# aarchiiive/diff-unet-amos

Measured on AMD Instinct MI355X. Metric: denoised voxel-steps/sec on 96^3 16-class AMOS patches, higher is better.
Workload: dtype f16

## Files before the change

diff_unet_amos_amd/csrc/common.hpp:

```cpp
#pragma once
#include <hip/hip_runtime.h>
#include <stdint.h>

namespace dua {
struct LdsAttr { const void* fn; int bytes; };
void register_lds_attrs(const LdsAttr* list, int n);
int ensure_prepared();
int device_cus();
struct LdsAttrs {
  template <int N> explicit LdsAttrs(const LdsAttr (&list)[N]) { register_lds_attrs(list, N); }
};


using f16 = _Float16;
typedef f16 f16x8 __attribute__((ext_vector_type(8)));
typedef f16 f16x4 __attribute__((ext_vector_type(4)));
typedef float f32x4 __attribute__((ext_vector_type(4)));
typedef float f32x16 __attribute__((ext_vector_type(16)));

enum : int { DT_F32 = 0, DT_F16 = 1 };

template <typename T> struct Elem;
template <> struct Elem<f16> {
  static constexpr int EPG = 8;
  using Frag = f16x8;
};
template <> struct Elem<float> {
  static constexpr int EPG = 4;
  using Frag = f32x4;
};

__device__ __forceinline__ void mma32(f32x16& acc, const f16x8& a, const f16x8& b) {
  acc = __builtin_amdgcn_mfma_f32_32x32x16_f16(a, b, acc, 0, 0, 0);
}
__device__ __forceinline__ void mma32(f32x16& acc, const f32x4& a, const f32x4& b) {
  acc = __builtin_amdgcn_mfma_f32_32x32x2f32(a[0], b[0], acc, 0, 0, 0);
  acc = __builtin_amdgcn_mfma_f32_32x32x2f32(a[1], b[1], acc, 0, 0, 0);
  acc = __builtin_amdgcn_mfma_f32_32x32x2f32(a[2], b[2], acc, 0, 0, 0);
  acc = __builtin_amdgcn_mfma_f32_32x32x2f32(a[3], b[3], acc, 0, 0, 0);
}

__device__ __forceinline__ float gelu_erf(float x) {
  const float z = fabsf(x) * 0.70710678118654752f;
  const float t = __builtin_amdgcn_rcpf(fmaf(0.3275911f, z, 1.f));
  float p = fmaf(t, 1.061405429f, -1.453152027f);
  p = fmaf(p, t, 1.421413741f);
  p = fmaf(p, t, -0.284496736f);
  p = fmaf(p, t, 0.254829592f);
  const float e = 1.f - p * t * __expf(-z * z);
  return 0.5f * x * (1.f + copysignf(e, x));
}

__device__ __forceinline__ float other_half(float v) {
  const auto pr = __builtin_amdgcn_permlane32_swap(__float_as_uint(v), __float_as_uint(v), false, false);
  return __uint_as_float((threadIdx.x & 32) ? pr[0] : pr[1]);
}

__device__ __forceinline__ long chan_off(bool blk, long v, int c, int stride, long nvox) {
  return blk ? ((long)(c >> 4) * nvox + v) * 16 + (c & 15) : v * stride + c;
}

__device__ __forceinline__ int acc_row(int i, int h) { return (i & 3) + 8 * (i >> 2) + 4 * h; }

__device__ __forceinline__ int xcd_remap(int bid, int n) {
  int q = n >> 3, r = n & 7, x = bid & 7, j = bid >> 3;
  return (x < r ? x * (q + 1) : r * (q + 1) + (x - r) * q) + j;
}

__device__ __forceinline__ void wide_tile_origin(int bid, int ntiles, int tiles_h, int tiles_w, int& d0, int& h0, int& w0) {
  const int per_slab = tiles_h * tiles_w;
  const int tile = xcd_remap(bid, ntiles);
  const int td = tile / per_slab, rem = tile - td * per_slab, th = rem / tiles_w, tw = rem - th * tiles_w;
  d0 = td * 8; h0 = th * 8; w0 = tw * 8;
}

__device__ __forceinline__ void lds_dma_16(const void* src_lane, unsigned lds_dst) {
  unsigned keep;
  asm volatile("s_mov_b32 %0, m0\n\ts_mov_b32 m0, %2\n\ts_nop 0\n\tglobal_load_lds_dwordx4 %1, off\n\ts_mov_b32 m0, %0"
               : "=&s"(keep) : "v"(src_lane), "s"(__builtin_amdgcn_readfirstlane(lds_dst)) : "memory");
}
__device__ __forceinline__ void lds_dma_16_m0_unsaved(const void* src_lane, unsigned lds_dst) {
  asm volatile("s_mov_b32 m0, %1\n\ts_nop 0\n\tglobal_load_lds_dwordx4 %0, off" : : "v"(src_lane), "s"(__builtin_amdgcn_readfirstlane(lds_dst)) : "memory");
}

constexpr int STAT_REPLICAS = 8;

using stat_t = long long;
constexpr int STAT_WORDS = 4;
constexpr double STAT_FRAC = 17592186044416.0;

struct InXform {
  const stat_t* stats;
  const float* gamma;
  const float* beta;
  const float* add;
  double inv_count;
  int add_stride, c_pad;
  float eps, slope;
};

__device__ __forceinline__ void stats_words_value(const stat_t (&w)[STAT_WORDS], double& S, double& Q) {
  S = (double)w[0] + (double)w[1] * (1.0 / STAT_FRAC);
  Q = (double)w[2] + (double)w[3] * (1.0 / STAT_FRAC);
}

__device__ __forceinline__ void stats_read(const stat_t* stats, int n, int c_pad, int c, double& S, double& Q) {
  stat_t w[STAT_WORDS] = {0, 0, 0, 0};
#pragma unroll
  for (int r = 0; r < STAT_REPLICAS; ++r) {
    const stat_t* p = stats + ((long)n * STAT_REPLICAS + r) * STAT_WORDS * c_pad + c;
#pragma unroll
    for (int k = 0; k < STAT_WORDS; ++k) w[k] += p[(long)k * c_pad];
  }
  stats_words_value(w, S, Q);
}

__device__ __forceinline__ void stats_words_to_sums(const stat_t (&v)[2 * STAT_WORDS], double& S, double& Q) {
  stat_t w[STAT_WORDS];
#pragma unroll
  for (int k = 0; k < STAT_WORDS; ++k) {
    w[k] = v[k] + v[STAT_WORDS + k];
    w[k] += __shfl_xor(w[k], 16);
    w[k] += __shfl_xor(w[k], 32);
  }
  stats_words_value(w, S, Q);
}

__device__ __forceinline__ void stats_read_wave16(const stat_t* stats, int n, int c_pad, int c, double& S, double& Q) {
  const int part = (threadIdx.x & 63) >> 4;
  const stat_t* p = stats + ((long)n * STAT_REPLICAS + 2 * part) * STAT_WORDS * c_pad + c;
  stat_t v[2 * STAT_WORDS];
#pragma unroll
  for (int k = 0; k < 2 * STAT_WORDS; ++k) v[k] = p[(long)k * c_pad];
#ifdef DUA_STATS_F64
  S = __longlong_as_double(v[0]) + __longlong_as_double(v[STAT_WORDS]);
  Q = __longlong_as_double(v[2]) + __longlong_as_double(v[STAT_WORDS + 2]);
  S += __shfl_xor(S, 16); S += __shfl_xor(S, 32);
  Q += __shfl_xor(Q, 16); Q += __shfl_xor(Q, 32);
#else
  stats_words_to_sums(v, S, Q);
#endif
}

__device__ __forceinline__ void norm_mean_rstd(double S, double Q, double inv_count, float eps, double& mean, float& rstd) {
  mean = S * inv_count;
  double var = Q * inv_count - mean * mean;
  var = var > 0 ? var : 0;
  rstd = (float)(1.0 / sqrt(var + (double)eps));
}
__device__ __forceinline__ void norm_scale_shift(double S, double Q, double inv_count, float eps, float gamma, float beta,
                                                 float& scale, float& shift) {
  double mean;
  float rstd;
  norm_mean_rstd(S, Q, inv_count, eps, mean, rstd);
  scale = gamma * rstd;
  shift = beta - (float)mean * scale;
}

__device__ __forceinline__ void xform_preamble(const InXform& xf, int n, int C, float* sc, float* sh, float* ad,
                                               int c_begin = 0) {
  if (!xf.stats) {
    for (int c = c_begin + threadIdx.x; c < C; c += blockDim.x) {
      sc[c] = 1.f; sh[c] = 0.f;
      ad[c] = xf.add ? xf.add[(long)n * xf.add_stride + c] : 0.f;
    }
    return;
  }
  const int lane = threadIdx.x & 63, wave = threadIdx.x >> 6, nw = blockDim.x >> 6;
  constexpr int UN = 4;
  for (int c0 = c_begin + wave * 16; c0 < C; c0 += UN * nw * 16) {
    double S[UN], Q[UN];
    float gam[UN], bet[UN], add[UN];
    int cc[UN];
#pragma unroll
    for (int u = 0; u < UN; ++u) {
      const int c = c0 + u * nw * 16 + (lane & 15);
      cc[u] = c < C ? c : C - 1;
      gam[u] = xf.gamma[cc[u]]; bet[u] = xf.beta[cc[u]];
      add[u] = xf.add ? xf.add[(long)n * xf.add_stride + cc[u]] : 0.f;
    }
#pragma unroll
    for (int u = 0; u < UN; ++u) {
      S[u] = 0; Q[u] = 0;
      if (c0 + u * nw * 16 < C) stats_read_wave16(xf.stats, n, xf.c_pad, cc[u], S[u], Q[u]);
    }
    const int part = lane >> 4;
    double Sm = S[0], Qm = Q[0];
    float gm = gam[0], bm = bet[0], am = add[0];
#pragma unroll
    for (int u = 1; u < UN; ++u)
      if (part == u) { Sm = S[u]; Qm = Q[u]; gm = gam[u]; bm = bet[u]; am = add[u]; }
    const int c = c0 + part * nw * 16 + (lane & 15);
    float g, b;
    norm_scale_shift(Sm, Qm, xf.inv_count, xf.eps, gm, bm, g, b);
    if (c0 + part * nw * 16 < C && c < C) {
      sc[c] = g;
      sh[c] = b;
      ad[c] = am;
    }
  }
}

}
#include "../../include/dua_hip.h"
namespace dua {
static inline InXform make_xform(const dua_in_norm* in, int C) {
  InXform x{};
  if (in && in->stats) {
    x.stats = in->stats; x.gamma = in->gamma; x.beta = in->beta; x.add = in->add;
    x.add_stride = in->add_stride > 0 ? in->add_stride : C;
    x.c_pad = in->c_pad; x.eps = in->eps;
    x.inv_count = in->count > 0 ? 1.0 / (double)in->count : 0.0;
  }
  x.slope = in ? in->slope : 0.f;
  return x;
}

__device__ __forceinline__ void stats_add(stat_t* stats, int n, int c_pad, int replica, int c, double S, double Q) {
  unsigned long long* p = (unsigned long long*)stats + ((long)n * STAT_REPLICAS + replica) * STAT_WORDS * c_pad + c;
#ifdef DUA_STATS_F64
  unsafeAtomicAdd((double*)p, S);
  unsafeAtomicAdd((double*)(p + 2L * c_pad), Q);
  return;
#endif
  constexpr double LIM = 4.0e18;
  constexpr double POISON = 140737488355328.0;
  if (!(fabs(S) < LIM) || !(fabs(Q) < LIM)) { S = POISON; Q = -POISON; }
  const double Si = rint(S), Qi = rint(Q);
  __hip_atomic_fetch_add(p, (unsigned long long)(long long)Si, __ATOMIC_RELAXED, __HIP_MEMORY_SCOPE_SYSTEM);
  __hip_atomic_fetch_add(p + c_pad, (unsigned long long)(long long)rint((S - Si) * STAT_FRAC), __ATOMIC_RELAXED, __HIP_MEMORY_SCOPE_SYSTEM);
  __hip_atomic_fetch_add(p + 2L * c_pad, (unsigned long long)(long long)Qi, __ATOMIC_RELAXED, __HIP_MEMORY_SCOPE_SYSTEM);
  __hip_atomic_fetch_add(p + 3L * c_pad, (unsigned long long)(long long)rint((Q - Qi) * STAT_FRAC), __ATOMIC_RELAXED, __HIP_MEMORY_SCOPE_SYSTEM);
}

template <typename T>
__device__ __forceinline__ void xform_prep(float* sc, float* sh, float* ad, float* sn, float slope) {
  if constexpr (sizeof(T) == 2) {
#pragma unroll
    for (int e = 0; e < Elem<T>::EPG; ++e) {
      sn[e] = slope * sc[e];
      const float b = sh[e] + ad[e];
      ad[e] = fmaf(slope, sh[e], ad[e]);
      sh[e] = b;
    }
  }
}

typedef unsigned u32x4_t __attribute__((ext_vector_type(4)));
__device__ __forceinline__ u32x4_t xform_frag_mix(u32x4_t x, const float* a, const float* b, const float* an, const float* bn) {
  u32x4_t p, n, r;
#pragma unroll
  for (int j = 0; j < 4; ++j) asm("v_fma_mixlo_f16 %0, %1, %2, %3 op_sel_hi:[1,0,0]" : "=v"(p[j]) : "v"(x[j]), "v"(a[2 * j]), "v"(b[2 * j]));
#pragma unroll
  for (int j = 0; j < 4; ++j) asm("v_fma_mixlo_f16 %0, %1, %2, %3 op_sel_hi:[1,0,0]" : "=v"(n[j]) : "v"(x[j]), "v"(an[2 * j]), "v"(bn[2 * j]));
#pragma unroll
  for (int j = 0; j < 4; ++j)
    asm("v_fma_mixhi_f16 %0, %1, %2, %3 op_sel:[1,0,0] op_sel_hi:[1,0,0]" : "+v"(p[j]) : "v"(x[j]), "v"(a[2 * j + 1]), "v"(b[2 * j + 1]));
#pragma unroll
  for (int j = 0; j < 4; ++j)
    asm("v_fma_mixhi_f16 %0, %1, %2, %3 op_sel:[1,0,0] op_sel_hi:[1,0,0]" : "+v"(n[j]) : "v"(x[j]), "v"(an[2 * j + 1]), "v"(bn[2 * j + 1]));
#pragma unroll
  for (int j = 0; j < 4; ++j) asm("v_pk_max_f16 %0, %1, %2" : "=v"(r[j]) : "v"(p[j]), "v"(n[j]));
  return r;
}

template <typename T>
__device__ __forceinline__ typename Elem<T>::Frag xform_frag(typename Elem<T>::Frag v, const float* sc, const float* sh,
                                                               const float* ad, const float* sn, float slope) {
  constexpr int E = Elem<T>::EPG;
  typename Elem<T>::Frag o;
  if constexpr (sizeof(T) == 2) {
    o = __builtin_bit_cast(typename Elem<T>::Frag, xform_frag_mix(__builtin_bit_cast(u32x4_t, v), sc, sh, sn, ad));
  } else {
#pragma unroll
    for (int j = 0; j < E; ++j) {
      float y = fmaf((float)v[j], sc[j], sh[j]);
      y = y > 0.f ? y : y * slope;
      o[j] = (T)(y + ad[j]);
    }
  }
  return o;
}

}
```

diff_unet_amos_amd/csrc/deconv.hip:

```cpp
#include "common.hpp"
#include "../../include/dua_hip.h"
#include "conv3_form.hpp"

namespace dua {



struct DeconvArgs {
  const void* x; const void* w; const float* bias; void* y;
  InXform xf;
  int N, D, H, W;
  int Cin, Cin_stride, Cin_off, Cout, Cout_stride, Cout_off;
  int nchunks, nct, lds_base;
  int out_blk;
  int Do, Ho, Wo;
  int pad;
};

template <typename F>
__device__ __forceinline__ void pad_copies(const DeconvArgs& a, long ov, F&& st) {
  const long hw = (long)a.Ho * a.Wo;
  const int od = (int)(ov / hw), oh = (int)((ov / a.Wo) % a.Ho), ow = (int)(ov % a.Wo);
  const int e = ((a.Do & 1) && od == a.Do - 2 ? 4 : 0) | ((a.Ho & 1) && oh == a.Ho - 2 ? 2 : 0) | ((a.Wo & 1) && ow == a.Wo - 2 ? 1 : 0);
  for (int c = 1; c < 8; ++c)
    if ((c & e) == c) st(ov + ((c & 4) ? hw : 0) + ((c & 2) ? a.Wo : 0) + (c & 1));
}

template <typename T>
__global__ __launch_bounds__(256) void deconv_k2s2_kernel(DeconvArgs a) {
  using namespace dc;
  using Frag = typename Elem<T>::Frag;
  constexpr int EPG = Elem<T>::EPG;
  constexpr int CK = KG * EPG;
  constexpr int OS = BN * (int)sizeof(T) + 16;
  extern __shared__ __attribute__((aligned(16))) char smem[];
  char* alds = smem;
  char* wlds = smem + A_BYTES;
  float* xsc = (float*)(smem + a.lds_base);
  float* xsh = xsc + a.nchunks * CK;
  float* xad = xsh + a.nchunks * CK;

  const int tid = threadIdx.x, lane = tid & 63, wave = tid >> 6, r = lane & 31, hh = lane >> 5;
  const long vox = (long)a.D * a.H * a.W;
  const long v0 = (long)blockIdx.x * TM;
  const int tap = blockIdx.y / a.nct, ct = blockIdx.y % a.nct, n = blockIdx.z;
  const T* xin = (const T*)a.x + (long)n * vox * a.Cin_stride + a.Cin_off;
  const char* wsrc = (const char*)a.w + ((long)tap * a.nct + ct) * a.nchunks * W_BYTES;

  f32x16 acc[2][2];
#pragma unroll
  for (int m = 0; m < 2; ++m)
#pragma unroll
    for (int q = 0; q < 2; ++q)
#pragma unroll
      for (int i = 0; i < 16; ++i) acc[m][q][i] = 0.f;

  const int kg_t = tid & 3;
  if (a.xf.stats != nullptr) xform_preamble(a.xf, n, a.Cin, xsc, xsh, xad);
  Frag pa[4];
  f32x4 pw;
  auto load_chunk = [&](int ch) {
    const int c0 = ch * CK + kg_t * EPG;
    const bool cok = c0 < a.Cin;
#pragma unroll
    for (int j = 0; j < 4; ++j) {
      const long v = v0 + (tid >> 2) + 64 * j;
      if (v < vox && cok) pa[j] = *(const Frag*)(xin + v * a.Cin_stride + c0);
      else
#pragma unroll
        for (int e = 0; e < EPG; ++e) pa[j][e] = (T)0.f;
    }
    pw = *(const f32x4*)(wsrc + (long)ch * W_BYTES + tid * 16);
  };
  load_chunk(0);
  for (int ch = 0; ch < a.nchunks; ++ch) {
    __syncthreads();
    const int c0 = ch * CK + kg_t * EPG;
    const bool xf = a.xf.stats != nullptr && c0 < a.Cin;
    float sc[EPG], sh[EPG], ad[EPG], sn[EPG];
    if (xf) {
#pragma unroll
      for (int e = 0; e < EPG; ++e) { sc[e] = xsc[c0 + e]; sh[e] = xsh[c0 + e]; ad[e] = xad[c0 + e]; }
      xform_prep<T>(sc, sh, ad, sn, a.xf.slope);
    }
#pragma unroll
    for (int j = 0; j < 4; ++j) {
      const int vl = (tid >> 2) + 64 * j;
      Frag f = pa[j];
      if (xf && v0 + vl < vox) f = xform_frag<T>(f, sc, sh, ad, sn, a.xf.slope);
      *(Frag*)(alds + vl * VS + kg_t * 16) = f;
    }
    *(f32x4*)(wlds + tid * 16) = pw;
    __syncthreads();
    if (ch + 1 < a.nchunks) load_chunk(ch + 1);
#pragma unroll
    for (int ks = 0; ks < KG / 2; ++ks) {
      Frag a0 = *(const Frag*)(alds + (wave * 64 + r) * VS + (2 * ks + hh) * 16);
      Frag a1 = *(const Frag*)(alds + (wave * 64 + 32 + r) * VS + (2 * ks + hh) * 16);
      Frag b0 = *(const Frag*)(wlds + ((2 * ks + hh) * BN + r) * 16);
      Frag b1 = *(const Frag*)(wlds + ((2 * ks + hh) * BN + 32 + r) * 16);
      mma32(acc[0][0], a0, b0);
      mma32(acc[0][1], a0, b1);
      mma32(acc[1][0], a1, b0);
      mma32(acc[1][1], a1, b1);
    }
  }
  __syncthreads();
  char* ot = smem + wave * 64 * OS;
#pragma unroll
  for (int q = 0; q < 2; ++q) {
    const int co = q * 32 + r;
    const float bq = a.bias[ct * BN + co];
#pragma unroll
    for (int m = 0; m < 2; ++m)
#pragma unroll
      for (int i = 0; i < 16; ++i)
        *(T*)(ot + (m * 32 + acc_row(i, hh)) * OS + co * (int)sizeof(T)) = (T)(acc[m][q][i] + bq);
  }
  __syncthreads();
  constexpr int GPV = BN / EPG, VPI = 64 / GPV;
  const int ti = tap >> 2, tj = (tap >> 1) & 1, tk = tap & 1;
  const int H2 = a.Ho, W2 = a.Wo;
  T* yout = (T*)a.y + (long)n * a.Do * H2 * W2 * a.Cout_stride + a.Cout_off + ct * BN;
#pragma unroll
  for (int it = 0; it < 64 / VPI; ++it) {
    const int vl = it * VPI + lane / GPV, cg = lane % GPV;
    const long v = v0 + wave * 64 + vl;
    if (v < vox && ct * BN + cg * EPG < a.Cout) {
      const int w = (int)(v % a.W); const long t = v / a.W;
      const int h = (int)(t % a.H), d = (int)(t / a.H);
      const long ov = ((long)(2 * d + ti) * H2 + (2 * h + tj)) * W2 + (2 * w + tk);
      const Frag o = *(const Frag*)(ot + vl * OS + cg * 16);
      *(Frag*)(yout + ov * a.Cout_stride + cg * EPG) = o;
      if (a.pad) pad_copies(a, ov, [&](long c) { *(Frag*)(yout + c * a.Cout_stride + cg * EPG) = o; });
    }
  }
}

template <typename T>
__global__ __launch_bounds__(256, 2) void deconv_k2s2_ksplit_kernel(DeconvArgs a) {
  using namespace dc;
  using namespace dcs;
  using Frag = typename Elem<T>::Frag;
  constexpr int EPG = Elem<T>::EPG;
  constexpr int CK = KG * EPG;
  extern __shared__ __attribute__((aligned(16))) char smem[];
  float* xsc = (float*)(smem + RED);
  float* xsh = xsc + a.nchunks * CK;
  float* xad = xsh + a.nchunks * CK;

  const int tid = threadIdx.x, lane = tid & 63, wave = tid >> 6, r = lane & 31, hh = lane >> 5;
  const long vox = (long)a.D * a.H * a.W;
  const long v0 = (long)blockIdx.x * TMS;
  const int tap = blockIdx.y / a.nct, ct = blockIdx.y % a.nct, n = blockIdx.z;
  const T* xin = (const T*)a.x + (long)n * vox * a.Cin_stride + a.Cin_off;
  const char* wsrc = (const char*)a.w + ((long)tap * a.nct + ct) * a.nchunks * W_BYTES;
  char* alds = smem + wave * STAGE;
  char* wlds = alds + TMS * VS;
  const int kg_t = lane & 3;
  const bool fused = a.xf.stats != nullptr;

  Frag pa[MC][4];
  f32x4 pw[MC][4];
#pragma unroll
  for (int c = 0; c < MC; ++c) {
    const int ch = wave + 4 * c;
    const int c0 = ch * CK + kg_t * EPG;
    const bool cok = ch < a.nchunks && c0 < a.Cin;
#pragma unroll
    for (int j = 0; j < 4; ++j) {
      const long v = v0 + (lane >> 2) + 16 * j;
      pa[c][j] = *(const Frag*)(xin + (v < vox && cok ? v * a.Cin_stride + c0 : 0));
      pw[c][j] = *(const f32x4*)(wsrc + (ch < a.nchunks ? (long)ch * W_BYTES + (lane + 64 * j) * 16 : 0));
    }
  }
  if (fused) xform_preamble(a.xf, n, a.Cin, xsc, xsh, xad);
  __syncthreads();

  f32x16 acc[2][2];
#pragma unroll
  for (int m = 0; m < 2; ++m)
#pragma unroll
    for (int q = 0; q < 2; ++q)
#pragma unroll
      for (int i = 0; i < 16; ++i) acc[m][q][i] = 0.f;
#pragma unroll
  for (int c = 0; c < MC; ++c) {
    const int ch = wave + 4 * c;
    if (ch >= a.nchunks) break;
    const int c0 = ch * CK + kg_t * EPG;
    const bool cok = c0 < a.Cin;
    float sc[EPG], sh[EPG], ad[EPG], sn[EPG];
    if (fused && cok) {
#pragma unroll
      for (int e = 0; e < EPG; ++e) { sc[e] = xsc[c0 + e]; sh[e] = xsh[c0 + e]; ad[e] = xad[c0 + e]; }
      xform_prep<T>(sc, sh, ad, sn, a.xf.slope);
    }
#pragma unroll
    for (int j = 0; j < 4; ++j) {
      const int vl = (lane >> 2) + 16 * j;
      const bool ok = v0 + vl < vox && cok;
      Frag f = pa[c][j];
      if (fused && cok) f = xform_frag<T>(f, sc, sh, ad, sn, a.xf.slope);
#pragma unroll
      for (int e = 0; e < EPG; ++e) f[e] = ok ? f[e] : (T)0.f;
      *(Frag*)(alds + vl * VS + kg_t * 16) = f;
      *(f32x4*)(wlds + (lane + 64 * j) * 16) = pw[c][j];
    }
    __builtin_amdgcn_fence(__ATOMIC_RELEASE, "wavefront");
    __builtin_amdgcn_wave_barrier();
    __builtin_amdgcn_fence(__ATOMIC_ACQUIRE, "wavefront");
#pragma unroll
    for (int ks = 0; ks < KG / 2; ++ks) {
      const Frag a0 = *(const Frag*)(alds + r * VS + (2 * ks + hh) * 16);
      const Frag a1 = *(const Frag*)(alds + (32 + r) * VS + (2 * ks + hh) * 16);
      const Frag b0 = *(const Frag*)(wlds + ((2 * ks + hh) * BN + r) * 16);
      const Frag b1 = *(const Frag*)(wlds + ((2 * ks + hh) * BN + 32 + r) * 16);
      mma32(acc[0][0], a0, b0);
      mma32(acc[0][1], a0, b1);
      mma32(acc[1][0], a1, b0);
      mma32(acc[1][1], a1, b1);
    }
    __builtin_amdgcn_fence(__ATOMIC_RELEASE, "wavefront");
    __builtin_amdgcn_wave_barrier();
    __builtin_amdgcn_fence(__ATOMIC_ACQUIRE, "wavefront");
  }
  __syncthreads();
  float* red = (float*)(smem + wave * TMS * RS);
#pragma unroll
  for (int m = 0; m < 2; ++m)
#pragma unroll
    for (int q = 0; q < 2; ++q)
#pragma unroll
      for (int i = 0; i < 16; ++i) red[(m * 32 + acc_row(i, hh)) * (RS / 4) + q * 32 + r] = acc[m][q][i];
  __syncthreads();
  const int ti = tap >> 2, tj = (tap >> 1) & 1, tk = tap & 1;
  const int H2 = a.Ho, W2 = a.Wo;
  T* yout = (T*)a.y + (long)n * a.Do * H2 * W2 * a.Cout_stride + a.Cout_off + ct * BN;
#pragma unroll
  for (int it = 0; it < 2; ++it) {
    const int item = tid + 256 * it, vl = item >> 3, cg = item & 7;
    float o[8];
#pragma unroll
    for (int e = 0; e < 8; ++e) o[e] = 0.f;
#pragma unroll
    for (int w = 0; w < 4; ++w) {
      const float* p = (const float*)(smem + w * TMS * RS) + vl * (RS / 4) + cg * 8;
      const f32x4 lo = *(const f32x4*)p, hi = *(const f32x4*)(p + 4);
#pragma unroll
      for (int e = 0; e < 4; ++e) { o[e] += lo[e]; o[4 + e] += hi[e]; }
    }
    const long v = v0 + vl;
    if (v < vox && ct * BN + cg * 8 < a.Cout) {
      const int w = (int)(v % a.W); const long t = v / a.W;
      const int h = (int)(t % a.H), d = (int)(t / a.H);
      const long ov = ((long)(2 * d + ti) * H2 + (2 * h + tj)) * W2 + (2 * w + tk);
      T* dst = yout + ov * a.Cout_stride + cg * 8;
      if constexpr (sizeof(T) == 2) {
        Frag f;
#pragma unroll
        for (int e = 0; e < 8; ++e) f[e] = (T)(o[e] + a.bias[ct * BN + cg * 8 + e]);
        *(Frag*)dst = f;
        if (a.pad) pad_copies(a, ov, [&](long c) { *(Frag*)(yout + c * a.Cout_stride + cg * 8) = f; });
      } else {
#pragma unroll
        for (int g = 0; g < 2; ++g) {
          Frag f;
#pragma unroll
          for (int e = 0; e < 4; ++e) f[e] = (T)(o[4 * g + e] + a.bias[ct * BN + cg * 8 + 4 * g + e]);
          *(Frag*)(dst + 4 * g) = f;
          if (a.pad) pad_copies(a, ov, [&](long c) { *(Frag*)(yout + c * a.Cout_stride + cg * 8 + 4 * g) = f; });
        }
      }
    }
  }
}

template <typename T, int MBLK>
__global__ __launch_bounds__(256) void deconv_k2s2_alltaps_kernel(DeconvArgs a) {
  using namespace dc;
  constexpr int TM = 64 * MBLK * 2, WR = 32 * MBLK;
  using Frag = typename Elem<T>::Frag;
  constexpr int EPG = Elem<T>::EPG;
  constexpr int CK = KG * EPG;
  constexpr int RB = 32 * (int)sizeof(T) + 16;
  constexpr int GPV = 32 / EPG, VPI = 64 / GPV, NST = 2 * WR / VPI;
  extern __shared__ __attribute__((aligned(16))) char smem[];
  const int VSA = a.nchunks * 64 + 16;
  char* alds = smem;
  char* wlds = alds + TM * VSA;
  char* stg = wlds + 4 * a.nchunks * W_BYTES;
  float* xsc = (float*)(stg + 2 * TM * RB);
  float* xsh = xsc + a.nchunks * CK;
  float* xad = xsh + a.nchunks * CK;

  const int tid = threadIdx.x, lane = tid & 63, wave = tid >> 6, r = lane & 31, hh = lane >> 5;
  const long vox = (long)a.D * a.H * a.W;
  const long v0 = (long)blockIdx.x * TM;
  const int ct = blockIdx.y, n = blockIdx.z;
  const T* xin = (const T*)a.x + (long)n * vox * a.Cin_stride + a.Cin_off;
  const int wtap = a.nchunks * W_BYTES;
  const char* wsrc = (const char*)a.w + (long)ct * wtap;
  const int kg_t = tid & 3;

  constexpr int MCH = 4;
  Frag f[MCH][TM / 64];
#pragma unroll
  for (int ch = 0; ch < MCH; ++ch) {
    const int c0 = ch * CK + kg_t * EPG;
    const bool cok = ch < a.nchunks && c0 < a.Cin;
#pragma unroll
    for (int j = 0; j < TM / 64; ++j) {
      const long v = v0 + (tid >> 2) + 64 * j;
      f[ch][j] = *(const Frag*)(xin + (v < vox && cok ? v * a.Cin_stride + c0 : 0));
    }
  }
  f32x4 wn[2][MCH];
  auto load_pair = [&](int tp) {
#pragma unroll
    for (int tk = 0; tk < 2; ++tk)
#pragma unroll
      for (int j = 0; j < MCH; ++j)
        wn[tk][j] = *(const f32x4*)(wsrc + (long)(2 * tp + tk) * a.nct * wtap + (j < a.nchunks ? (tid + 256 * j) * 16 : 0));
  };
  auto store_pair = [&](int tp) {
#pragma unroll
    for (int tk = 0; tk < 2; ++tk)
#pragma unroll
      for (int j = 0; j < MCH; ++j)
        if (j < a.nchunks) *(f32x4*)(wlds + ((tp & 1) * 2 + tk) * wtap + (tid + 256 * j) * 16) = wn[tk][j];
  };
  load_pair(0);
  if (a.xf.stats != nullptr) {
    xform_preamble(a.xf, n, a.Cin, xsc, xsh, xad);
    __syncthreads();
  }
#pragma unroll
  for (int ch = 0; ch < MCH; ++ch) {
    if (ch >= a.nchunks) break;
    const int c0 = ch * CK + kg_t * EPG;
    const bool cok = c0 < a.Cin;
    const bool xf = a.xf.stats != nullptr && cok;
    float sc[EPG], sh[EPG], ad[EPG], sn[EPG];
    if (xf) {
#pragma unroll
      for (int e = 0; e < EPG; ++e) { sc[e] = xsc[c0 + e]; sh[e] = xsh[c0 + e]; ad[e] = xad[c0 + e]; }
      xform_prep<T>(sc, sh, ad, sn, a.xf.slope);
    }
#pragma unroll
    for (int j = 0; j < TM / 64; ++j) {
      const int vl = (tid >> 2) + 64 * j;
      const bool ok = v0 + vl < vox && cok;
      Frag g = f[ch][j];
      if (xf) g = xform_frag<T>(g, sc, sh, ad, sn, a.xf.slope);
#pragma unroll
      for (int e = 0; e < EPG; ++e) g[e] = ok ? g[e] : (T)0.f;
      *(Frag*)(alds + vl * VSA + ch * 64 + kg_t * 16) = g;
    }
  }
  store_pair(0);
  __syncthreads();

  const int H2 = a.Ho, W2 = a.Wo;
  const long ovox = (long)a.Do * H2 * W2;
  T* yout = (T*)a.y + (long)n * ovox * a.Cout_stride;
  const float bq0 = a.bias[ct * BN + r], bq1 = a.bias[ct * BN + 32 + r];
  char* ot = stg + wave * 2 * WR * RB;
  int ovb[NST];
#pragma unroll
  for (int it = 0; it < NST; ++it) {
    const int j = it * VPI + lane / GPV;
    const long v = v0 + wave * WR + (j >> 1);
    const int vi = (int)(v < vox ? v : 0);
    const int w = vi % a.W, t = vi / a.W, h = t % a.H, d = t / a.H;
    ovb[it] = v < vox ? ((2 * d) * H2 + 2 * h) * W2 + 2 * w + (j & 1) : -1;
  }
  load_pair(1);
  for (int tp = 0; tp < 4; ++tp) {
    f32x16 acc[2][MBLK][2];
#pragma unroll
    for (int tk = 0; tk < 2; ++tk) {
#pragma unroll
      for (int m = 0; m < MBLK; ++m)
#pragma unroll
        for (int i = 0; i < 16; ++i) { acc[tk][m][0][i] = bq0; acc[tk][m][1][i] = bq1; }
      const char* wb = wlds + ((tp & 1) * 2 + tk) * wtap;
      for (int ch = 0; ch < a.nchunks; ++ch) {
#pragma unroll
        for (int ks = 0; ks < KG / 2; ++ks) {
          const Frag b0 = *(const Frag*)(wb + ch * W_BYTES + ((2 * ks + hh) * BN + r) * 16);
          const Frag b1 = *(const Frag*)(wb + ch * W_BYTES + ((2 * ks + hh) * BN + 32 + r) * 16);
#pragma unroll
          for (int m = 0; m < MBLK; ++m) {
            const Frag am = *(const Frag*)(alds + (wave * WR + m * 32 + r) * VSA + ch * 64 + (2 * ks + hh) * 16);
            mma32(acc[tk][m][0], am, b0);
            mma32(acc[tk][m][1], am, b1);
          }
        }
      }
    }
    if (tp < 3) store_pair(tp + 1);
    if (tp < 2) load_pair(tp + 2);
    const int toff = ((tp >> 1) * H2 + (tp & 1)) * W2;
#pragma unroll
    for (int q = 0; q < 2; ++q) {
#pragma unroll
      for (int tk = 0; tk < 2; ++tk)
#pragma unroll
        for (int m = 0; m < MBLK; ++m)
#pragma unroll
          for (int i = 0; i < 16; ++i)
            *(T*)(ot + (2 * (m * 32 + acc_row(i, hh)) + tk) * RB + r * (int)sizeof(T)) = (T)acc[tk][m][q][i];
      __builtin_amdgcn_wave_barrier();
#pragma unroll
      for (int it = 0; it < NST; ++it) {
        const int j = it * VPI + lane / GPV, cg = lane % GPV;
        if (ovb[it] >= 0 && ct * BN + q * 32 + cg * EPG < a.Cout) {
          const Frag o = *(const Frag*)(ot + j * RB + cg * 16);
          const int c0 = a.Cout_off + ct * BN + q * 32 + cg * EPG;
          *(Frag*)(yout + chan_off(a.out_blk, ovb[it] + toff, c0, a.Cout_stride, ovox)) = o;
          if (a.pad) pad_copies(a, ovb[it] + toff, [&](long c) { *(Frag*)(yout + chan_off(a.out_blk, c, c0, a.Cout_stride, ovox)) = o; });
        }
      }
      __builtin_amdgcn_wave_barrier();
    }
    __syncthreads();
  }
}

struct DeconvResArgs {
  DeconvArgs base;
  const void* xs; const void* ws; stat_t* stats;
  int Cs, Cs_stride, Cs_off, cout_pad;
};

template <int NSK>
__global__ __launch_bounds__(256, 2) void deconv_k2s2_res_kernel(DeconvResArgs ra) {
  using namespace dc;
  using T = f16;
  const DeconvArgs& a = ra.base;
  constexpr int TM = 128, WR = 32, EPG = 8;
  using Frag = f16x8;
  constexpr int RB = 32 * 2 + 16;
  constexpr int GPV = 4, VPI = 16, NST = 2 * WR / VPI;
  extern __shared__ __attribute__((aligned(16))) char smem[];
  const int VSA = a.nchunks * 64 + 16;
  char* alds = smem;
  char* wlds = alds + TM * VSA;
  char* stg = wlds + 4 * a.nchunks * W_BYTES;
  char* skw = stg + 2 * TM * RB;

  const int tid = threadIdx.x, lane = tid & 63, wave = tid >> 6, r = lane & 31, hh = lane >> 5;
  const long vox = (long)a.D * a.H * a.W;
  const long v0 = (long)blockIdx.x * TM;
  const int ct = blockIdx.y, n = blockIdx.z;
  const T* xin = (const T*)a.x + (long)n * vox * a.Cin_stride + a.Cin_off;
  const int wtap = a.nchunks * W_BYTES;
  const char* wsrc = (const char*)a.w + (long)ct * wtap;
  const int kg_t = tid & 3;
  const int H2 = 2 * a.H, W2 = 2 * a.W;
  const T* xsk = (const T*)ra.xs + (long)n * vox * 8 * ra.Cs_stride + ra.Cs_off;

  constexpr int MCH = 4;
  Frag f[MCH][TM / 64];
#pragma unroll
  for (int ch = 0; ch < MCH; ++ch) {
    const int c0 = ch * 32 + kg_t * EPG;
    const bool cok = ch < a.nchunks && c0 < a.Cin;
#pragma unroll
    for (int j = 0; j < TM / 64; ++j) {
      const long v = v0 + (tid >> 2) + 64 * j;
      f[ch][j] = *(const Frag*)(xin + (v < vox && cok ? v * a.Cin_stride + c0 : 0));
    }
  }
  f32x4 wn[2][MCH];
  auto load_pair = [&](int tp) {
#pragma unroll
    for (int tk = 0; tk < 2; ++tk)
#pragma unroll
// ... 261 lines not shown
```

diff_unet_amos_amd/csrc/instnorm.hip:

```cpp
#include "common.hpp"
#include "../../include/dua_hip.h"

namespace dua {

__global__ void instnorm_finalize_kernel(InXform xf, int C, float* scale, float* shift) {
  extern __shared__ float sm[];
  const int n = blockIdx.x;
  xform_preamble(xf, n, C, sm, sm + C, sm + 2 * C);
  __syncthreads();
  for (int c = threadIdx.x; c < C; c += blockDim.x) { scale[n * C + c] = sm[c]; shift[n * C + c] = sm[C + c]; }
}

template <typename T, bool POOL, bool EMB, bool ODD = false>
__global__ __launch_bounds__(256) void materialize_kernel(const T* __restrict__ raw, int C, int raw_stride,
                                                          InXform xf,
                                                          const T* __restrict__ emb, int emb_stride, T* __restrict__ out,
                                                          int out_stride, int out_off, T* __restrict__ pooled,
                                                          int pool_stride, int D, int H, int W, long total, int out_blk) {
  using Frag = typename Elem<T>::Frag;
  constexpr int EPG = Elem<T>::EPG;
  extern __shared__ float sm[];
  const int gpc = C / EPG;
  const int n = blockIdx.y;
  const float slope = xf.slope;
  xform_preamble(xf, n, C, sm, sm + C, sm + 2 * C);
  __syncthreads();
  const long vox_n = (long)D * H * W;
  const bool fixed = 256 % gpc == 0;
  float sc[EPG], sh[EPG], ad[EPG];
  if (fixed) {
    const int cg = threadIdx.x % gpc;
#pragma unroll
    for (int e = 0; e < EPG; ++e) { sc[e] = sm[cg * EPG + e]; sh[e] = sm[C + cg * EPG + e]; ad[e] = sm[2 * C + cg * EPG + e]; }
  }
  for (long it = blockIdx.x * 256L + threadIdx.x; it < total; it += (long)gridDim.x * 256) {
    const int cg = (int)(it % gpc);
    long v = it / gpc;
    if (!fixed) {
#pragma unroll
      for (int e = 0; e < EPG; ++e) { sc[e] = sm[cg * EPG + e]; sh[e] = sm[C + cg * EPG + e]; ad[e] = sm[2 * C + cg * EPG + e]; }
    }
    if constexpr (!POOL) {
      const long gv = n * vox_n + v;
      Frag x = *(const Frag*)(raw + gv * raw_stride + cg * EPG);
      Frag o;
      Frag ev;
      if constexpr (EMB) ev = *(const Frag*)(emb + gv * emb_stride + cg * EPG);
#pragma unroll
      for (int e = 0; e < EPG; ++e) {
        float y = fmaf((float)x[e], sc[e], sh[e]);
        y = (y > 0.f ? y : y * slope) + ad[e];
        if constexpr (EMB) y += (float)ev[e];
        o[e] = (T)y;
      }
      *(Frag*)(out + n * vox_n * out_stride + chan_off(out_blk, v, out_off + cg * EPG, out_stride, vox_n)) = o;
    } else {
      const int W2 = W >> 1, H2 = H >> 1;
      const int WB = ODD ? (W + 1) >> 1 : W2, HB = ODD ? (H + 1) >> 1 : H2;
      const int pw = (int)(v % WB); v /= WB;
      const int ph = (int)(v % HB); const int pd = (int)(v / HB);
      float mx[EPG];
#pragma unroll
      for (int e = 0; e < EPG; ++e) mx[e] = -INFINITY;
      long gvk[8];
      bool okk[8];
      Frag xk[8], evk[EMB ? 8 : 1];
#pragma unroll
      for (int k = 0; k < 8; ++k) {
        const int d = 2 * pd + (k >> 2), h = 2 * ph + ((k >> 1) & 1), w = 2 * pw + (k & 1);
        okk[k] = !ODD || (d < D && h < H && w < W);
        gvk[k] = n * vox_n + (okk[k] ? ((long)d * H + h) * W + w : 0);
        xk[k] = *(const Frag*)(raw + gvk[k] * raw_stride + cg * EPG);
      }
      if constexpr (EMB) {
#pragma unroll
        for (int k = 0; k < 8; ++k) evk[k] = *(const Frag*)(emb + gvk[k] * emb_stride + cg * EPG);
      }
      __builtin_amdgcn_sched_barrier(0);
#pragma unroll
      for (int k = 0; k < 8; ++k) {
        Frag o;
#pragma unroll
        for (int e = 0; e < EPG; ++e) {
          float y = fmaf((float)xk[k][e], sc[e], sh[e]);
          y = (y > 0.f ? y : y * slope) + ad[e];
          if constexpr (EMB) y += (float)evk[k][e];
          o[e] = (T)y;
          mx[e] = fmaxf(mx[e], (float)o[e]);
        }
        if (okk[k])
          *(Frag*)(out + n * vox_n * out_stride + chan_off(out_blk, gvk[k] - n * vox_n, out_off + cg * EPG, out_stride, vox_n)) = o;
      }
      if (ODD && (pd >= (D >> 1) || ph >= H2 || pw >= W2)) continue;
      Frag po;
#pragma unroll
      for (int e = 0; e < EPG; ++e) po[e] = (T)mx[e];
      const long pv = n * (ODD ? (long)(D >> 1) * H2 * W2 : vox_n >> 3) + ((long)pd * H2 + ph) * W2 + pw;
      *(Frag*)(pooled + pv * pool_stride + cg * EPG) = po;
    }
  }
}

template <typename T>
static int launch_materialize(const dua_materialize_desc* d, const void* raw, const dua_in_norm* in,
                              const void* emb, void* out, void* pooled, hipStream_t s) {
  constexpr int EPG = Elem<T>::EPG;
  const long vox = (long)d->D * d->H * d->W;
  const bool pool = pooled != nullptr;
  const bool odd = pool && ((d->D | d->H | d->W) & 1);
  const long blocks3 = odd ? (long)((d->D + 1) / 2) * ((d->H + 1) / 2) * ((d->W + 1) / 2) : vox / 8;
  const long total = (pool ? blocks3 : vox) * (d->C / EPG);
  long blocks = (total + 255) / 256;
  if (blocks > 8192) blocks = 8192;
  dim3 grid((unsigned)blocks, d->N);
  const InXform xf = make_xform(in, d->C);
  const size_t lds = 3 * sizeof(float) * d->C;
  auto go = [&](auto kern) {
    hipLaunchKernelGGL(kern, grid, dim3(256), lds, s, (const T*)raw, d->C, d->raw_stride, xf, (const T*)emb, d->emb_stride,
                       (T*)out, d->out_stride, d->out_off, (T*)pooled, pool ? d->pool_stride : 0, d->D, d->H, d->W, total, d->out_blocked ? 1 : 0);
  };
  if (odd) { if (emb) go(materialize_kernel<T, true, true, true>); else go(materialize_kernel<T, true, false, true>); }
  else if (pool) { if (emb) go(materialize_kernel<T, true, true>); else go(materialize_kernel<T, true, false>); }
  else { if (emb) go(materialize_kernel<T, false, true>); else go(materialize_kernel<T, false, false>); }
  return (int)hipGetLastError();
}

}

extern "C" {

int dua_instnorm_finalize(int N, int C, const dua_in_norm* in, float* scale, float* shift, void* stream) {
  if (N <= 0 || C <= 0 || !in || !in->stats || !in->gamma || !in->beta || in->c_pad < C || !scale || !shift)
    return DUA_ERR_ARG;
  hipLaunchKernelGGL(dua::instnorm_finalize_kernel, dim3(N), dim3(256), 3 * sizeof(float) * C, (hipStream_t)stream,
                     dua::make_xform(in, C), C, scale, shift);
  return (int)hipGetLastError();
}

int dua_materialize(const dua_materialize_desc* d, const void* raw, const dua_in_norm* in,
                    const void* emb, void* out, void* pooled, void* stream) {
  if (!d || !raw || !in || !in->stats || !in->gamma || !in->beta || in->c_pad < d->C || !out) return DUA_ERR_ARG;
  if (d->C % 8 || d->raw_stride % 8 || d->out_stride % 8 || d->out_off % 8 || (emb && d->emb_stride % 8)) return DUA_ERR_ARG;
  if (pooled && (d->D == 1 || d->H == 1 || d->W == 1 || d->pool_stride % 8)) return DUA_ERR_ARG;
  if (d->out_blocked && (d->dtype != DUA_F16 || d->out_stride % 16 || d->out_off % 16 || d->C % 16)) return DUA_ERR_ARG;
  if (d->dtype == DUA_F16) return dua::launch_materialize<dua::f16>(d, raw, in, emb, out, pooled, (hipStream_t)stream);
  if (d->dtype == DUA_F32) return dua::launch_materialize<float>(d, raw, in, emb, out, pooled, (hipStream_t)stream);
  return DUA_ERR_ARG;
}

}
```

Before: 678.9 million.

## Add channel-sliced materialize kernel for small grids; hoist deconv norm preamble

```diff
diff --git a/diff_unet_amos_amd/csrc/common.hpp b/diff_unet_amos_amd/csrc/common.hpp
--- a/diff_unet_amos_amd/csrc/common.hpp
+++ b/diff_unet_amos_amd/csrc/common.hpp
@@ -157,6 +157,7 @@
   shift = beta - (float)mean * scale;
 }
 
+template <bool ALL_GROUPS = false>
 __device__ __forceinline__ void xform_preamble(const InXform& xf, int n, int C, float* sc, float* sh, float* ad,
                                                int c_begin = 0) {
   if (!xf.stats) {
@@ -182,7 +183,8 @@
 #pragma unroll
     for (int u = 0; u < UN; ++u) {
       S[u] = 0; Q[u] = 0;
-      if (c0 + u * nw * 16 < C) stats_read_wave16(xf.stats, n, xf.c_pad, cc[u], S[u], Q[u]);
+      if (ALL_GROUPS || c0 + u * nw * 16 < C)
+        stats_read_wave16(xf.stats, n, xf.c_pad, cc[u], S[u], Q[u]);
     }
     const int part = lane >> 4;
     double Sm = S[0], Qm = Q[0];
diff --git a/diff_unet_amos_amd/csrc/deconv.hip b/diff_unet_amos_amd/csrc/deconv.hip
--- a/diff_unet_amos_amd/csrc/deconv.hip
+++ b/diff_unet_amos_amd/csrc/deconv.hip
@@ -160,6 +160,7 @@
   const int kg_t = lane & 3;
   const bool fused = a.xf.stats != nullptr;
 
+  if (fused) xform_preamble<true>(a.xf, n, a.Cin, xsc, xsh, xad);
   Frag pa[MC][4];
   f32x4 pw[MC][4];
 #pragma unroll
@@ -174,7 +175,6 @@
       pw[c][j] = *(const f32x4*)(wsrc + (ch < a.nchunks ? (long)ch * W_BYTES + (lane + 64 * j) * 16 : 0));
     }
   }
-  if (fused) xform_preamble(a.xf, n, a.Cin, xsc, xsh, xad);
   __syncthreads();
 
   f32x16 acc[2][2];
diff --git a/diff_unet_amos_amd/csrc/instnorm.hip b/diff_unet_amos_amd/csrc/instnorm.hip
--- a/diff_unet_amos_amd/csrc/instnorm.hip
+++ b/diff_unet_amos_amd/csrc/instnorm.hip
@@ -11,21 +11,97 @@
   for (int c = threadIdx.x; c < C; c += blockDim.x) { scale[n * C + c] = sm[c]; shift[n * C + c] = sm[C + c]; }
 }
 
+template <typename T>
+struct MatArgs {
+  const T* raw; int C, raw_stride;
+  InXform xf;
+  const T* emb; int emb_stride;
+  T* out; int out_stride, out_off;
+  T* pooled; int pool_stride;
+  int D, H, W;
+  long total;
+  int out_blk;
+};
+
+template <typename T, bool POOL, bool EMB, bool ODD, typename Index>
+__device__ __forceinline__ void materialize_item(const MatArgs<T>& a, int n, Index v, int cg, bool live,
+                                                 const float (&sc)[Elem<T>::EPG], const float (&sh)[Elem<T>::EPG],
+                                                 const float (&ad)[Elem<T>::EPG]) {
+  using Frag = typename Elem<T>::Frag;
+  constexpr int EPG = Elem<T>::EPG;
+  const float slope = a.xf.slope;
+  const int D = a.D, H = a.H, W = a.W;
+  const long vox_n = (long)D * H * W;
+  if constexpr (!POOL) {
+    const long gv = n * vox_n + v;
+    Frag x = *(const Frag*)(a.raw + gv * a.raw_stride + cg * EPG);
+    Frag o;
+    Frag ev;
+    if constexpr (EMB) ev = *(const Frag*)(a.emb + gv * a.emb_stride + cg * EPG);
+#pragma unroll
+    for (int e = 0; e < EPG; ++e) {
+      float y = fmaf((float)x[e], sc[e], sh[e]);
+      y = (y > 0.f ? y : y * slope) + ad[e];
+      if constexpr (EMB) y += (float)ev[e];
+      o[e] = (T)y;
+    }
+    if (live)
+      *(Frag*)(a.out + n * vox_n * a.out_stride + chan_off(a.out_blk, v, a.out_off + cg * EPG, a.out_stride, vox_n)) = o;
+  } else {
+    const int W2 = W >> 1, H2 = H >> 1;
+    const int WB = ODD ? (W + 1) >> 1 : W2, HB = ODD ? (H + 1) >> 1 : H2;
+    const int pw = (int)(v % WB); v /= WB;
+    const int ph = (int)(v % HB); const int pd = (int)(v / HB);
+    float mx[EPG];
+#pragma unroll
+    for (int e = 0; e < EPG; ++e) mx[e] = -INFINITY;
+    long gvk[8];
+    bool okk[8];
+    Frag xk[8], evk[EMB ? 8 : 1];
+#pragma unroll
+    for (int k = 0; k < 8; ++k) {
+      const int d = 2 * pd + (k >> 2), h = 2 * ph + ((k >> 1) & 1), w = 2 * pw + (k & 1);
+      okk[k] = !ODD || (d < D && h < H && w < W);
+      gvk[k] = n * vox_n + (okk[k] ? ((long)d * H + h) * W + w : 0);
+      xk[k] = *(const Frag*)(a.raw + gvk[k] * a.raw_stride + cg * EPG);
+    }
+    if constexpr (EMB) {
+#pragma unroll
+      for (int k = 0; k < 8; ++k) evk[k] = *(const Frag*)(a.emb + gvk[k] * a.emb_stride + cg * EPG);
+    }
+    __builtin_amdgcn_sched_barrier(0);
+#pragma unroll
+    for (int k = 0; k < 8; ++k) {
+      Frag o;
+#pragma unroll
+      for (int e = 0; e < EPG; ++e) {
+        float y = fmaf((float)xk[k][e], sc[e], sh[e]);
+        y = (y > 0.f ? y : y * slope) + ad[e];
+        if constexpr (EMB) y += (float)evk[k][e];
+        o[e] = (T)y;
+        mx[e] = fmaxf(mx[e], (float)o[e]);
+      }
+      if (live && okk[k])
+        *(Frag*)(a.out + n * vox_n * a.out_stride +
+                 chan_off(a.out_blk, gvk[k] - n * vox_n, a.out_off + cg * EPG, a.out_stride, vox_n)) = o;
+    }
+    if (!live || (ODD && (pd >= (D >> 1) || ph >= H2 || pw >= W2))) return;
+    Frag po;
+#pragma unroll
+    for (int e = 0; e < EPG; ++e) po[e] = (T)mx[e];
+    const long pv = n * (ODD ? (long)(D >> 1) * H2 * W2 : vox_n >> 3) + ((long)pd * H2 + ph) * W2 + pw;
+    *(Frag*)(a.pooled + pv * a.pool_stride + cg * EPG) = po;
+  }
+}
+
 template <typename T, bool POOL, bool EMB, bool ODD = false>
-__global__ __launch_bounds__(256) void materialize_kernel(const T* __restrict__ raw, int C, int raw_stride,
-                                                          InXform xf,
-                                                          const T* __restrict__ emb, int emb_stride, T* __restrict__ out,
-                                                          int out_stride, int out_off, T* __restrict__ pooled,
-                                                          int pool_stride, int D, int H, int W, long total, int out_blk) {
-  using Frag = typename Elem<T>::Frag;
+__global__ __launch_bounds__(256) void materialize_kernel(MatArgs<T> a) {
   constexpr int EPG = Elem<T>::EPG;
   extern __shared__ float sm[];
-  const int gpc = C / EPG;
+  const int C = a.C, gpc = C / EPG;
   const int n = blockIdx.y;
-  const float slope = xf.slope;
-  xform_preamble(xf, n, C, sm, sm + C, sm + 2 * C);
+  xform_preamble(a.xf, n, C, sm, sm + C, sm + 2 * C);
   __syncthreads();
-  const long vox_n = (long)D * H * W;
   const bool fixed = 256 % gpc == 0;
   float sc[EPG], sh[EPG], ad[EPG];
   if (fixed) {
@@ -33,73 +109,45 @@
 #pragma unroll
     for (int e = 0; e < EPG; ++e) { sc[e] = sm[cg * EPG + e]; sh[e] = sm[C + cg * EPG + e]; ad[e] = sm[2 * C + cg * EPG + e]; }
   }
-  for (long it = blockIdx.x * 256L + threadIdx.x; it < total; it += (long)gridDim.x * 256) {
+  for (long it = blockIdx.x * 256L + threadIdx.x; it < a.total; it += (long)gridDim.x * 256) {
     const int cg = (int)(it % gpc);
-    long v = it / gpc;
     if (!fixed) {
 #pragma unroll
       for (int e = 0; e < EPG; ++e) { sc[e] = sm[cg * EPG + e]; sh[e] = sm[C + cg * EPG + e]; ad[e] = sm[2 * C + cg * EPG + e]; }
     }
-    if constexpr (!POOL) {
-      const long gv = n * vox_n + v;
-      Frag x = *(const Frag*)(raw + gv * raw_stride + cg * EPG);
-      Frag o;
-      Frag ev;
-      if constexpr (EMB) ev = *(const Frag*)(emb + gv * emb_stride + cg * EPG);
-#pragma unroll
-      for (int e = 0; e < EPG; ++e) {
-        float y = fmaf((float)x[e], sc[e], sh[e]);
-        y = (y > 0.f ? y : y * slope) + ad[e];
-        if constexpr (EMB) y += (float)ev[e];
-        o[e] = (T)y;
-      }
-      *(Frag*)(out + n * vox_n * out_stride + chan_off(out_blk, v, out_off + cg * EPG, out_stride, vox_n)) = o;
-    } else {
-      const int W2 = W >> 1, H2 = H >> 1;
-      const int WB = ODD ? (W + 1) >> 1 : W2, HB = ODD ? (H + 1) >> 1 : H2;
-      const int pw = (int)(v % WB); v /= WB;
-      const int ph = (int)(v % HB); const int pd = (int)(v / HB);
-      float mx[EPG];
-#pragma unroll
-      for (int e = 0; e < EPG; ++e) mx[e] = -INFINITY;
-      long gvk[8];
-      bool okk[8];
-      Frag xk[8], evk[EMB ? 8 : 1];
-#pragma unroll
-      for (int k = 0; k < 8; ++k) {
-        const int d = 2 * pd + (k >> 2), h = 2 * ph + ((k >> 1) & 1), w = 2 * pw + (k & 1);
-        okk[k] = !ODD || (d < D && h < H && w < W);
-        gvk[k] = n * vox_n + (okk[k] ? ((long)d * H + h) * W + w : 0);
-        xk[k] = *(const Frag*)(raw + gvk[k] * raw_stride + cg * EPG);
-      }
-      if constexpr (EMB) {
-#pragma unroll
-        for (int k = 0; k < 8; ++k) evk[k] = *(const Frag*)(emb + gvk[k] * emb_stride + cg * EPG);
-      }
-      __builtin_amdgcn_sched_barrier(0);
-#pragma unroll
-      for (int k = 0; k < 8; ++k) {
-        Frag o;
-#pragma unroll
-        for (int e = 0; e < EPG; ++e) {
-          float y = fmaf((float)xk[k][e], sc[e], sh[e]);
-          y = (y > 0.f ? y : y * slope) + ad[e];
-          if constexpr (EMB) y += (float)evk[k][e];
-          o[e] = (T)y;
-          mx[e] = fmaxf(mx[e], (float)o[e]);
-        }
-        if (okk[k])
-          *(Frag*)(out + n * vox_n * out_stride + chan_off(out_blk, gvk[k] - n * vox_n, out_off + cg * EPG, out_stride, vox_n)) = o;
-      }
-      if (ODD && (pd >= (D >> 1) || ph >= H2 || pw >= W2)) continue;
-      Frag po;
-#pragma unroll
-      for (int e = 0; e < EPG; ++e) po[e] = (T)mx[e];
-      const long pv = n * (ODD ? (long)(D >> 1) * H2 * W2 : vox_n >> 3) + ((long)pd * H2 + ph) * W2 + pw;
-      *(Frag*)(pooled + pv * pool_stride + cg * EPG) = po;
-    }
-  }
-}
+    materialize_item<T, POOL, EMB, ODD>(a, n, it / gpc, cg, true, sc, sh, ad);
+  }
+}
+
+template <typename T, bool POOL, bool EMB, bool ODD = false>
+__global__ __launch_bounds__(256) void materialize_sliced_kernel(MatArgs<T> a) {
+  constexpr int EPG = Elem<T>::EPG;
+  extern __shared__ float sm[];
+  const int slice_c = blockDim.x / 4;
+  const int C = a.C, gpc = C / EPG, gps = slice_c / EPG;
+  const int n = blockIdx.y, c0 = blockIdx.z * slice_c;
+  const int cg = c0 / EPG + threadIdx.x % gps;
+  const int v = blockIdx.x * (blockDim.x / gps) + threadIdx.x / gps;
+  const bool live = v < (int)(a.total / gpc);
+  float sc[EPG], sh[EPG], ad[EPG];
+  {
+    const int lane = threadIdx.x & 63, c = c0 + (threadIdx.x >> 6) * 16 + (lane & 15);
+    const float gam = a.xf.gamma[c], bet = a.xf.beta[c];
+    const float add = a.xf.add ? a.xf.add[(long)n * a.xf.add_stride + c] : 0.f;
+    double S, Q;
+    stats_read_wave16(a.xf.stats, n, a.xf.c_pad, c, S, Q);
+    float g, b;
+    norm_scale_shift(S, Q, a.xf.inv_count, a.xf.eps, gam, bet, g, b);
+    if (lane < 16) { sm[c] = g; sm[C + c] = b; sm[2 * C + c] = add; }
+  }
+  __syncthreads();
+#pragma unroll
+  for (int e = 0; e < EPG; ++e) { sc[e] = sm[cg * EPG + e]; sh[e] = sm[C + cg * EPG + e]; ad[e] = sm[2 * C + cg * EPG + e]; }
+  materialize_item<T, POOL, EMB, ODD>(a, n, live ? v : 0, cg, live, sc, sh, ad);
+}
+
+constexpr long MAT_SLICED_BELOW = 128;
+constexpr int MAT_SLICE_THREADS = 256, MAT_SLICE_C = MAT_SLICE_THREADS / 4;
 
 template <typename T>
 static int launch_materialize(const dua_materialize_desc* d, const void* raw, const dua_in_norm* in,
@@ -112,16 +160,24 @@
   const long total = (pool ? blocks3 : vox) * (d->C / EPG);
   long blocks = (total + 255) / 256;
   if (blocks > 8192) blocks = 8192;
-  dim3 grid((unsigned)blocks, d->N);
-  const InXform xf = make_xform(in, d->C);
+  MatArgs<T> a{(const T*)raw, d->C, d->raw_stride, make_xform(in, d->C), (const T*)emb, d->emb_stride, (T*)out, d->out_stride,
+               d->out_off, (T*)pooled, pool ? d->pool_stride : 0, d->D, d->H, d->W, total, d->out_blocked ? 1 : 0};
   const size_t lds = 3 * sizeof(float) * d->C;
-  auto go = [&](auto kern) {
-    hipLaunchKernelGGL(kern, grid, dim3(256), lds, s, (const T*)raw, d->C, d->raw_stride, xf, (const T*)emb, d->emb_stride,
-                       (T*)out, d->out_stride, d->out_off, (T*)pooled, pool ? d->pool_stride : 0, d->D, d->H, d->W, total, d->out_blocked ? 1 : 0);
-  };
-  if (odd) { if (emb) go(materialize_kernel<T, true, true, true>); else go(materialize_kernel<T, true, false, true>); }
-  else if (pool) { if (emb) go(materialize_kernel<T, true, true>); else go(materialize_kernel<T, true, false>); }
-  else { if (emb) go(materialize_kernel<T, false, true>); else go(materialize_kernel<T, false, false>); }
+  using Kern = void (*)(MatArgs<T>);
+  const int variant = (odd ? 4 : pool ? 2 : 0) + (emb ? 1 : 0);
+  if (blocks < MAT_SLICED_BELOW && d->C % MAT_SLICE_C == 0) {
+    static const Kern sliced[6] = {materialize_sliced_kernel<T, false, false>,      materialize_sliced_kernel<T, false, true>,
+                                   materialize_sliced_kernel<T, true, false>,       materialize_sliced_kernel<T, true, true>,
+                                   materialize_sliced_kernel<T, true, false, true>, materialize_sliced_kernel<T, true, true, true>};
+    const long items = total / (d->C / EPG), per_wg = MAT_SLICE_THREADS / (MAT_SLICE_C / EPG);
+    hipLaunchKernelGGL(sliced[variant], dim3((unsigned)((items + per_wg - 1) / per_wg), d->N, d->C / MAT_SLICE_C),
+                       dim3(MAT_SLICE_THREADS), lds, s, a);
+  } else {
+    static const Kern full[6] = {materialize_kernel<T, false, false>,      materialize_kernel<T, false, true>,
+                                 materialize_kernel<T, true, false>,       materialize_kernel<T, true, true>,
+                                 materialize_kernel<T, true, false, true>, materialize_kernel<T, true, true, true>};
+    hipLaunchKernelGGL(full[variant], dim3((unsigned)blocks, d->N), dim3(256), lds, s, a);
+  }
   return (int)hipGetLastError();
 }
 
```

Result: no change. 680.6 million, median of 2 (+0.3%).
